# kaushik87599/Melo-GAN

Measured on AMD Instinct MI355X. Metric: piano-roll samples/sec (G+D step), batch=64 128x256 roll, higher is better.
Workload: dtype f32; 1 GPU; cfg2: 128x256 piano-roll, batch=64 per GPU, full G+D+emotion-D step (1 critic update incl. gradient penalty + 1 generator update); global_batch=64, T=256, C=128, parallelism=dp1, graph=True

## Files before the change

### include/melo_gan_hip.h

```cpp
#ifndef MELO_GAN_HIP_H
#define MELO_GAN_HIP_H

#include <stddef.h>
#include <stdint.h>

#ifdef __cplusplus
extern "C" {
#endif

typedef void* mg_stream_t;

enum { MG_ACT_NONE = 0, MG_ACT_RELU = 1, MG_ACT_LRELU = 2, MG_ACT_GELU = 3, MG_ACT_TANH = 4 };

typedef struct mg_epilogue {
    const float* bias;
    const float* scale;
    const float* shift;
    float* zout;
    int act;
    const float* gref;
    int gact;
    const float* emul;
    const float* gscale;
    int accumulate;
// ... 12 lines not shown
                       int B, int Tin, int Cin, int N, int Tout,
                       int w_sn, int w_sc, long xbs, long ybs,
                       const mg_epilogue* epi, void* work, size_t work_bytes, mg_stream_t stream);

int mg_wq_relayout(const float* w, float* wq, int N, int Cc, int K, int w_sn, int w_sc, mg_stream_t stream);
int mg_conv16_supported(int B, int Tin, int Cin, int N, int transposed, int Tout);
int mg_conv16_plan(int B, int Tin, int N, int transposed, int* batch_rows_per_tile, int* part_rows, int* tile_rows);
int mg_conv16_poolable(int B, int Tin, int Cin, int N);
typedef struct mg_conv16_extra {
    float* part;
    float* pool;
    float pool_scale;
    int y_perm;
    const float* mix_real;
    const float* mix_alpha;
    float* mix_out;
    int mix_rows;
    const float* bnb_a;
    const float* bnb_z;
    const float* bnb_mean;
    const float* bnb_invstd;
    double* bnb_part;
    int bnb_act;
} mg_conv16_extra;
int mg_conv16(const float* x, const float* wq, float* y, int B, int Tin, int Cin, int N, int transposed, int Tout,
              long xbs, long ybs, const mg_epilogue* epi, const mg_conv16_extra* extra , mg_stream_t stream);
int mg_bn_train_bwd_parts(const double* part, int part_rows, const float* da, const float* a, const float* z, float* dz, long R,
                          int C, const float* gamma, const float* beta, const float* save_mean, const float* save_invstd,
                          float* dgamma, float* dbeta, int act, mg_stream_t stream);
int mg_bn_train_fwd_parts(const float* part, int part_rows_per_group, int groups, const float* z, float* a, long R, int C,
                          const float* gamma, const float* beta, float* running_mean, float* running_var, float momentum,
                          float eps, float* save_mean, float* save_invstd, int act, mg_stream_t stream);

#define MG_CHAIN_MAX_OPS 16
#define MG_CHAIN_SLOTS 6
#define MG_CHAIN_MAX_VEC 512
enum { MG_CH_LOAD = 1, MG_CH_STORE = 2, MG_CH_LAYERNORM = 3, MG_CH_LIN_FWD = 4, MG_CH_LIN_DGRAD = 5, MG_CH_SOFTMAX_CE = 6,
       MG_CH_DHEAD = 7, MG_CH_MEAN_T = 8, MG_CH_COPY = 9 };
typedef struct mg_chain_op {
    int kind;
    int a, b;
    int n0, n1;
    int act;
    int i0, i1;
    float f0;
    const float* p0; long ld0;
    const float* p1; long ld1;
// ... 347 lines not shown
```

### melo-gan_amd/_lib.py

```python
import ctypes as C
import os

_HERE = os.path.dirname(os.path.abspath(__file__))
LIB_PATH = os.path.join(_HERE, "libmelogan_hip.so")
if os.environ.get("MELO_LIB_VARIANT"):
    LIB_PATH = os.path.join(os.path.dirname(_HERE), "tools", "_build", "libmelogan_" + os.environ["MELO_LIB_VARIANT"] + ".so")

ACT_NONE, ACT_RELU, ACT_LRELU, ACT_GELU, ACT_TANH = 0, 1, 2, 3, 4

vp, i32, i64, f32, sz = C.c_void_p, C.c_int, C.c_long, C.c_float, C.c_size_t


class Epilogue(C.Structure):
    _fields_ = [("bias", vp), ("scale", vp), ("shift", vp), ("zout", vp), ("act", i32),
                ("gref", vp), ("gact", i32), ("emul", vp), ("gscale", vp), ("accumulate", i32)]


class EpilogueBf16(C.Structure):
    _fields_ = [("scale", vp), ("shift", vp), ("zout", vp), ("act", i32), ("gref", vp), ("gact", i32), ("gscale", vp),
                ("accumulate", i32)]


class Conv16Extra(C.Structure):
    _fields_ = [("part", vp), ("pool", vp), ("pool_scale", f32), ("y_perm", i32), ("mix_real", vp), ("mix_alpha", vp),
                ("mix_out", vp), ("mix_rows", i32), ("bnb_a", vp), ("bnb_z", vp), ("bnb_mean", vp), ("bnb_invstd", vp),
                ("bnb_part", vp), ("bnb_act", i32)]


class ChainOp(C.Structure):
    _fields_ = [("kind", i32), ("a", i32), ("b", i32), ("n0", i32), ("n1", i32), ("act", i32), ("i0", i32), ("i1", i32), ("f0", f32),
                ("p0", vp), ("ld0", i64), ("p1", vp), ("ld1", i64), ("p2", vp), ("ld2", i64), ("p3", vp), ("ld3", i64),
                ("q0", vp), ("lq0", i64), ("q1", vp), ("lq1", i64), ("t0", vp)]


CH_LOAD, CH_STORE, CH_LAYERNORM, CH_LIN_FWD, CH_LIN_DGRAD, CH_SOFTMAX_CE, CH_DHEAD, CH_MEAN_T, CH_COPY = 1, 2, 3, 4, 5, 6, 7, 8, 9
CHAIN_MAX_OPS, CHAIN_SLOTS, CHAIN_MAX_VEC = 16, 6, 512


class StageJob(C.Structure):
    _fields_ = [("src", vp), ("dst", vp), ("idx", vp), ("row_bytes", i64), ("src_rows", i64), ("dst_pitch", i64), ("rows", i64)]


MAX_STAGE_JOBS = 8


class Augment(C.Structure):
    _fields_ = [("program", i32), ("noise_std", f32), ("dropout_prob", f32), ("pitch_shift_prob", f32), ("tempo_jitter", f32),
                ("note_dropout", f32), ("velocity_jitter", f32), ("timing_jitter", f32), ("pitch_shift", i32), ("seed", C.c_uint64)]

# ... 37 lines not shown

class Voice(C.Structure):
    _fields_ = [("n_partials", i32), ("mult", C.c_uint32 * VOICE_MAX_PARTIALS), ("weight", f32 * VOICE_MAX_PARTIALS),
                ("decay", f32 * VOICE_MAX_PARTIALS), ("attack", i32), ("release_tau", f32), ("release_len", i32), ("fs", f32)]


class MlpCls(C.Structure):
    _fields_ = [("n_hidden", i32), ("in_dim", i32), ("width", i32 * MLP_MAX_HIDDEN), ("n_classes", i32),
                ("w", vp * (MLP_MAX_HIDDEN + 1)), ("b", vp * (MLP_MAX_HIDDEN + 1)), ("z", vp * MLP_MAX_HIDDEN),
                ("a", vp * MLP_MAX_HIDDEN), ("dz", vp * MLP_MAX_HIDDEN), ("mask", vp * MLP_MAX_HIDDEN)]


SIGNATURES = {
    "mg_version": (i32, []),
    "mg_last_error": (C.c_char_p, []),
    "mg_conv_workspace_bytes": (sz, [i32, i32, i32]),
    "mg_conv1d_gather": (i32, [vp, vp, vp, i32, i32, i32, i32, i32, i32, i32, i32, i32, i64, i64, C.POINTER(Epilogue), vp, sz, i64, vp]),
    "mg_conv1d_scatter2": (i32, [vp, vp, vp, i32, i32, i32, i32, i32, i32, i32, i64, i64, C.POINTER(Epilogue), vp, sz, vp]),
    "mg_wq_relayout": (i32, [vp, vp, i32, i32, i32, i32, i32, vp]),
    "mg_conv16_supported": (i32, [i32, i32, i32, i32, i32, i32]),
    "mg_conv16_plan": (i32, [i32, i32, i32, i32, C.POINTER(i32), C.POINTER(i32), C.POINTER(i32)]),
    "mg_conv16": (i32, [vp, vp, vp, i32, i32, i32, i32, i32, i32, i64, i64, C.POINTER(Epilogue), C.POINTER(Conv16Extra), vp]),
    "mg_conv16_poolable": (i32, [i32, i32, i32, i32]),
    "mg_bn_train_fwd_parts": (i32, [vp, i32, i32, vp, vp, i64, i32, vp, vp, vp, vp, f32, f32, vp, vp, i32, vp]),
    "mg_linear_workspace_bytes": (sz, [i32, i32, i32]),
    "mg_linear": (i32, [vp, vp, vp, i32, i32, i32, i32, i32, C.POINTER(Epilogue), i32, vp, sz, vp]),
    "mg_conv_tile_config": (i32, [i64, i32, i32]),
    "mg_conv_plan": (i32, [i32, i32, i32, i32, i32, i32, i32, i32, sz, C.POINTER(i32), C.POINTER(i32)]),
    "mg_conv_finish_vec": (i32, [i32, i64, i32]),
    "mg_linear_route": (i32, [i32, i32, i32, i32, i32, i32, i32, i32, C.POINTER(i32), C.POINTER(i32), C.POINTER(i32)]),
    "mg_conv_thin_route": (i32, [vp, i64, i32, i32, i32, i32, i32]),
    "mg_wb_relayout": (i32, [vp, vp, i32, i32, i32, i32, i32, i32, vp]),
    "mg_conv1d_s1_bf16_supported": (i32, [i32, i32, i32, i32, i32]),
    "mg_conv1d_s1_bf16": (i32, [vp, i32, vp, vp, i32, i32, i32, i32, i32, i32, C.POINTER(EpilogueBf16), vp]),
    "mg_meanT_fwd_bf16": (i32, [vp, vp, i32, i32, i32, vp]),
    "mg_meanT_bwd_bf16": (i32, [vp, vp, vp, i32, vp, i32, i32, i32, vp]),
    "mg_wgrad_workspace_bytes": (sz, [i32, i32, i32, i32, i32]),
    "mg_wgrad": (i32, [vp, vp, i32, vp, vp, i32, vp, vp, i32, i32, i32, i32, i32, i32, i32, vp, sz, vp]),
    "mg_wgrad_multi": (i32, [vp, i32, i32, i32, vp, sz, vp]),
    "mg_colsum_workspace_bytes": (sz, [i32]),
    "mg_colsum": (i32, [vp, i64, i32, vp, vp, vp, sz, vp]),
    "mg_bn_workspace_bytes": (sz, [i32, i32]),
    "mg_bn_train_fwd": (i32, [vp, vp, i64, i32, i32, vp, vp, vp, vp, f32, f32, vp, vp, i32, vp, sz, vp]),
    "mg_bn_train_bwd": (i32, [vp, vp, vp, vp, i64, i32, vp, vp, vp, vp, vp, vp, i32, vp, sz, vp]),
    "mg_bn_train_bwd_parts": (i32, [vp, i32, vp, vp, vp, vp, i64, i32, vp, vp, vp, vp, vp, vp, i32, vp]),
    "mg_bn_eval_fwd": (i32, [vp, vp, i64, i32, vp, vp, vp, vp, f32, i32, vp]),
# ... 134 lines not shown
```

### melo-gan_amd/csrc/conv16_mfma.hip

```cpp
#include "common.h"
#include <stdlib.h>
#include <type_traits>

namespace {

typedef unsigned u32x4 __attribute__((ext_vector_type(4)));

struct Conv16P {
    const float* x;
    const float* wq;
    float* y;
    int B, Tin, Cin, Tm, Tout, N;
    long xbs, ybs;
    int x_bytes, w_bytes;
    int tt_log2, n_ttiles;
    unsigned nt_magic;
    mg_epilogue e;
    float* part;
    float* pool;
    float pool_scale;
    int y_perm;
    const float* mix_real;
    const float* mix_alpha;
    float* mix_out;
    int mix_rows;
    const float* bnb_a;
    const float* bnb_z;
    const float* bnb_mean;
    const float* bnb_invstd;
    double* bnb_part;
    int bnb_act;
};

constexpr int K5 = 5;
constexpr int BKC = 16;
template <bool TR2> struct PitchOf { static constexpr int value = TR2 ? 24 : 20; };
constexpr int BN = 32;
constexpr int WPLANE = BN * 4;
constexpr int WSLAB = 4 * K5 * WPLANE;
constexpr int MAXX = 3;
constexpr int NWU = 3;

template <bool TR2, int RT, bool RID>
__global__ __launch_bounds__(256, 2) void conv16_kernel(const Conv16P p) {
    constexpr int BM = 32 * RT;
    constexpr int SX = PitchOf<TR2>::value;
    constexpr int SA = TR2 ? 1 : 2;
    constexpr int NR = TR2 ? 3 : 5;
    constexpr int NPH = TR2 ? 2 : 1;
    extern __shared__ __attribute__((aligned(16))) float smem[];

    const int tid = threadIdx.x, lane = tid & 63, wave = tid >> 6;
    const int wm = wave >> 1, wn = wave & 1;
    const int li = lane & 15, kq = lane >> 4;
    const int TT = 1 << p.tt_log2, TB = BM >> p.tt_log2;
    const int R = (TT - 1) * SA + NR;
    const int nrows = TB * R;
    const int xs_floats = nrows * SX;
    const int buf_floats = xs_floats + WSLAB;

    const int mtile = blockIdx.x;
    int mq = (int)__umulhi((unsigned)mtile, p.nt_magic);
    if ((mq + 1) * p.n_ttiles <= mtile) ++mq;
    const int b0 = mq * TB;
    const int t0 = (mtile - mq * p.n_ttiles) * TT;
    const int n0 = blockIdx.y * BN;
    const int tin0 = TR2 ? (t0 - 1) : (2 * t0 - 2);

    auto lds4 = [&](int off) { return reinterpret_cast<f32x4*>(__builtin_assume_aligned(smem + off, 16)); };

    int abase[RT];
#pragma unroll
    for (int rt = 0; rt < RT; ++rt) {
        const int im = (wm * RT + rt) * 16 + li;
        const int seg = im >> p.tt_log2, tl = im & (TT - 1);
        abase[rt] = (seg * R + tl * SA) * SX + 4 * kq;
    }
    const int bbase = xs_floats + kq * K5 * WPLANE + (16 * wn + li) * 4;

    constexpr int KA = RT == 1 ? 2 : 1;
    f32x4 acc[NPH][RT][KA];
#pragma unroll
    for (int ph = 0; ph < NPH; ++ph)
#pragma unroll
        for (int rt = 0; rt < RT; ++rt)
#pragma unroll
            for (int ka = 0; ka < KA; ++ka) acc[ph][rt][ka] = f32x4{0.f, 0.f, 0.f, 0.f};

    const __amdgpu_buffer_rsrc_t xrsrc = __builtin_amdgcn_make_buffer_rsrc(const_cast<float*>(p.x), 0, p.x_bytes, 0x00020000);
    const __amdgpu_buffer_rsrc_t wrsrc = __builtin_amdgcn_make_buffer_rsrc(const_cast<float*>(p.wq), 0, p.w_bytes, 0x00020000);
    const int sink = 2 * buf_floats + 4 * tid;
    constexpr int NST = MAXX + NWU;
    unsigned so[NST];
    int sl[NST], sd[NST];
#pragma unroll
    for (int j = 0; j < MAXX; ++j) {
        const int idx = tid + 256 * j;
        so[j] = 0x80000000u;
        sl[j] = sink;
        sd[j] = 0;
        if (idx < nrows * 4) {
            const int row = idx >> 2, q = idx & 3;
            const int seg = (TB == 1) ? 0 : row / R, r = row - seg * R;
            const int b = b0 + seg, tin = tin0 + r;
            sl[j] = row * SX + 4 * q;
            sd[j] = buf_floats;
            if (b < p.B && tin >= 0 && tin < p.Tin)
                so[j] = ((unsigned)b * (unsigned)p.xbs + (unsigned)(tin * p.Cin + 4 * q)) * 4u;
        }
    }
#pragma unroll
    for (int i = 0; i < NWU; ++i) {
        const int u = tid + 256 * i;
        so[MAXX + i] = 0x80000000u;
        sl[MAXX + i] = sink;
        sd[MAXX + i] = 0;
        if (u < 4 * K5 * BN) {
            const int pl = u >> 5, n = u & 31;
            sl[MAXX + i] = xs_floats + u * 4;
            sd[MAXX + i] = buf_floats;
            if (n0 + n < p.N) so[MAXX + i] = ((unsigned)pl * (unsigned)p.N + (unsigned)(n0 + n)) * 16u;
        }
    }
    const unsigned wchunk = (unsigned)(K5 * p.N) * 16u;
    f32x4 sr[NST];
    auto bload = [&](const __amdgpu_buffer_rsrc_t& rsrc, unsigned voff, unsigned soff) {
        const u32x4 v = __builtin_amdgcn_raw_buffer_load_b128(rsrc, voff, soff, 0);
// ... 51 lines not shown
#pragma unroll
        for (int u = 0; u < NST; ++u) store_unit(u, 0);
        const int c1 = min(BKC, c_last);
#pragma unroll
        for (int u = 0; u < NST; ++u) load_unit(u, 4u * (unsigned)c1, (unsigned)(c1 >> 2) * wchunk);
        __syncthreads();
#pragma unroll
        for (int g = 0; g < NFR; ++g) frag_piece(0, 0, g, fa[0], fb[0]);
    }
    for (int c0 = 0;;) {
        chunk(std::integral_constant<int, 0>{}, min(c0 + 2 * BKC, c_last));
        c0 += BKC;
        if (c0 >= p.Cin) break;
        chunk(std::integral_constant<int, 1>{}, min(c0 + 2 * BKC, c_last));
        c0 += BKC;
        if (c0 >= p.Cin) break;
    }

    const mg_epilogue& E = p.e;
    const int n = n0 + 16 * wn + li;
    if (n >= p.N) return;
    const float bias = E.bias ? E.bias[n] : 0.f;
    const float scale = E.scale ? E.scale[n] : 1.f, shift = E.scale ? E.shift[n] : 0.f;
    const float gscale = E.gscale ? E.gscale[n] : 1.f;
    float st1 = 0.f, cnt = 0.f;
    double bs1 = 0.0, bs2 = 0.0;
    const float bnb_mu = (RID && p.bnb_part) ? p.bnb_mean[n] : 0.f, bnb_is = (RID && p.bnb_part) ? p.bnb_invstd[n] : 0.f;
    const bool want_stats = RID && (p.part || p.pool);
#pragma unroll
    for (int rt = 0; rt < RT; ++rt)
#pragma unroll
        for (int ph = 0; ph < NPH; ++ph) {
            f32x4 a = acc[ph][rt][0];
            if constexpr (KA == 2) a += acc[ph][rt][1];
            unsigned di[4], yi[4];
            bool ok[4], mixrow[4];
            int brow[4];
#pragma unroll
            for (int r = 0; r < 4; ++r) {
                const int im = (wm * RT + rt) * 16 + 4 * kq + r;
                const int seg = im >> p.tt_log2, tl = im & (TT - 1);
                const int b = b0 + seg, t = t0 + tl;
                const int tout = TR2 ? 2 * t + ph : t;
                di[r] = (unsigned)((b * p.Tout + tout) * p.N + n);
                yi[r] = (unsigned)(b * (int)p.ybs + ((RID && p.y_perm) ? n * p.Tout + tout : tout * p.N + n));
                ok[r] = b < p.B && t < p.Tm && tout < p.Tout;
// ... 111 lines not shown
            float m2 = 0.f;
#pragma unroll
            for (int rt = 0; rt < RT; ++rt)
#pragma unroll
                for (int ph = 0; ph < NPH; ++ph)
#pragma unroll
                    for (int r = 0; r < 4; ++r) {
                        const int im = (wm * RT + rt) * 16 + 4 * kq + r;
                        const int seg = im >> p.tt_log2, tl = im & (TT - 1);
                        const int b = b0 + seg, t = t0 + tl;
                        const int tout = TR2 ? 2 * t + ph : t;
                        const float d = acc[ph][rt][0][r] - mw;
                        if (b < p.B && t < p.Tm && tout < p.Tout) m2 += d * d;
                    }
            m2 += __shfl_xor(m2, 16, 64); m2 += __shfl_xor(m2, 32, 64);
            if (kq == 0) {
                float* dst = p.part + (long)(2 * blockIdx.x + wm) * 3 * p.N + n;
                dst[0] = st1;
                dst[p.N] = m2;
                dst[2 * p.N] = cnt;
            }
        }
    }
}

__global__ void wq_relayout_kernel(const float* __restrict__ w, float* __restrict__ wq, int N, int Cc, int K, int sn, int sc) {
    const long i = (long)blockIdx.x * blockDim.x + threadIdx.x;
    if (i >= (long)N * Cc * K) return;
    const int e = (int)(i & 3);
    const long r = i >> 2;
    const int n = (int)(r % N);
    const long r2 = r / N;
    const int k = (int)(r2 % K), q = (int)(r2 / K);
    wq[i] = w[(long)n * sn + (long)(4 * q + e) * sc + k];
}

template <bool TR2, int RT, bool RID>
int launch16(Conv16P p, hipStream_t stream) {
    constexpr int BM = 32 * RT;
    constexpr int SX = PitchOf<TR2>::value;
    constexpr int SA = TR2 ? 1 : 2;
    constexpr int NR = TR2 ? 3 : 5;
    int lg = mg_ilog2_ceil(p.Tm);
    const int lgbm = mg_ilog2_ceil(BM);
    if (lg > lgbm) lg = lgbm;
    p.tt_log2 = lg;
    const int TT = 1 << lg, TB = BM >> lg;
    p.n_ttiles = (int)mg_cdiv(p.Tm, TT);
    p.nt_magic = p.n_ttiles > 1 ? (unsigned)((1ULL << 32) / (unsigned)p.n_ttiles) : 0xFFFFFFFFu;
    const int R = (TT - 1) * SA + NR;
    if (TB * R * 4 > 256 * MAXX) return MG_EUNSUP;
    const size_t lds = 2 * ((size_t)TB * R * SX + WSLAB) * sizeof(float) + 256 * 4 * sizeof(float);
    auto kernel = &conv16_kernel<TR2, RT, RID>;
    static std::atomic<uint64_t> optin;
    if (int rc = mg_lds_optin(reinterpret_cast<const void*>(kernel), optin)) return rc;
    dim3 grid((unsigned)(p.n_ttiles * mg_cdiv(p.B, TB)), (unsigned)mg_cdiv(p.N, BN));
    hipLaunchKernelGGL(kernel, grid, dim3(256), lds, stream, p);
    MG_CHECK_LAUNCH("conv16");
    return MG_OK;
}

}

extern "C" int mg_wq_relayout(const float* w, float* wq, int N, int Cc, int K, int w_sn, int w_sc, mg_stream_t stream) {
    MG_CHECK_ARG(w && wq && N > 0 && Cc > 0 && K > 0 && Cc % 4 == 0 && w_sn > 0 && w_sc > 0, "mg_wq_relayout: bad args");
    const long total = (long)N * Cc * K;
    hipLaunchKernelGGL(wq_relayout_kernel, dim3((unsigned)mg_cdiv(total, 256)), dim3(256), 0, (hipStream_t)stream, w, wq, N, Cc, K,
                       w_sn, w_sc);
    MG_CHECK_LAUNCH("wq_relayout");
    return MG_OK;
}

static int pick_rt(long m_rows, int N) {
    if (const char* f = getenv("MG_CONV16_RT")) return atoi(f) == 1 ? 1 : 2;
    auto balance = [](long n) { return n >= 1024 ? 1.0 : (double)n / (double)(mg_cdiv(n, 256) * 256); };
    const long n2 = mg_cdiv(m_rows, 64) * mg_cdiv(N, BN), n1 = mg_cdiv(m_rows, 32) * mg_cdiv(N, BN);
    return balance(n1) > balance(n2) + 0.1 ? 1 : 2;
}

extern "C" int mg_conv16_supported(int B, int Tin, int Cin, int N, int transposed, int Tout) {
    if (B <= 0 || Tin <= 0 || Cin % BKC || N % BN) return 0;
    const int Tm = transposed ? Tin : (Tin + 4 - K5) / 2 + 1;
    if (Tm < 4) return 0;
    if (transposed && !(Tout == 2 * Tin || Tout == 2 * Tin - 1)) return 0;
// ... 4 lines not shown
    if (lg > mg_ilog2_ceil(BM)) lg = mg_ilog2_ceil(BM);
    const int TT = 1 << lg, TB = BM >> lg, R = (TT - 1) * (transposed ? 1 : 2) + (transposed ? 3 : 5);
    return TB * R * 4 <= 256 * MAXX;
}

extern "C" int mg_conv16_plan(int B, int Tin, int N, int transposed, int* batch_rows_per_tile, int* part_rows, int* tile_rows) {
    const int Tm = transposed ? Tin : (Tin + 4 - K5) / 2 + 1;
    const int BM = 32 * pick_rt((long)B * Tm, N);
    int lg = mg_ilog2_ceil(Tm);
    if (lg > mg_ilog2_ceil(BM)) lg = mg_ilog2_ceil(BM);
    const int TT = 1 << lg, TB = BM >> lg;
    if (batch_rows_per_tile) *batch_rows_per_tile = TB;
    if (tile_rows) *tile_rows = BM;
    if (part_rows) *part_rows = 2 * (int)(mg_cdiv(Tm, TT) * mg_cdiv(B, TB));
    return MG_OK;
}

extern "C" int mg_conv16_poolable(int B, int Tin, int Cin, int N) {
    if (!mg_conv16_supported(B, Tin, Cin, N, 0, 0)) return 0;
    const int Tm = (Tin + 4 - K5) / 2 + 1;
    return Tm == 16 * pick_rt((long)B * Tm, N);
}

extern "C" int mg_conv16(const float* x, const float* wq, float* y, int B, int Tin, int Cin, int N, int transposed, int Tout,
                         long xbs, long ybs, const mg_epilogue* epi, const mg_conv16_extra* extra, mg_stream_t stream) {
    const mg_conv16_extra ex = extra ? *extra : mg_conv16_extra{};
    float* const part = ex.part;
    float* const pool = ex.pool;
    const float pool_scale = ex.pool_scale;
    MG_CHECK_ARG(x && wq && y, "mg_conv16: null tensor");
    MG_CHECK_ARG(!(part && epi && epi->accumulate), "mg_conv16: statistics of an accumulating launch are not defined");
    MG_CHECK_ARG(!(pool && epi && epi->accumulate), "mg_conv16: the mean of an accumulating launch is not defined");
    MG_CHECK_ARG(!pool || (!transposed && mg_conv16_poolable(B, Tin, Cin, N)), "mg_conv16: shape is not poolable");
    MG_CHECK_ARG(!ex.mix_out || (ex.mix_real && ex.mix_alpha && ex.mix_rows > 0 && ex.mix_rows <= B && !ex.y_perm),
                 "mg_conv16: mix needs real, alpha, 0 < rows <= B and the plain output order");
    MG_CHECK_ARG(!ex.y_perm || (ybs == 0 || ybs == (long)N * (transposed ? Tout : (Tin + 4 - K5) / 2 + 1)),
                 "mg_conv16: the permuted output order needs a dense y");
    const int Tm = transposed ? Tin : (Tin + 4 - K5) / 2 + 1;
    if (!transposed) Tout = Tm;
    MG_CHECK_ARG(mg_conv16_supported(B, Tin, Cin, N, transposed, Tout), "mg_conv16: unsupported shape B=%d Tin=%d Cin=%d N=%d", B, Tin, Cin, N);
    Conv16P p{};
    p.x = x; p.wq = wq; p.y = y;
    p.B = B; p.Tin = Tin; p.Cin = Cin; p.Tm = Tm; p.Tout = Tout; p.N = N;
    p.xbs = xbs ? xbs : (long)Tin * Cin;
    p.ybs = ybs ? ybs : (long)Tout * N;
    const long xb = ((long)(B - 1) * p.xbs + (long)Tin * Cin) * 4, yb = (long)(B - 1) * p.ybs + (long)Tout * N;
    MG_CHECK_ARG(xb < (1L << 31) && yb < (1L << 31) && p.ybs < (1L << 31), "mg_conv16: tensor exceeds the 2^31 limit");
    p.x_bytes = (int)xb;
    p.w_bytes = (int)((long)N * Cin * K5 * 4);
// ... 31 lines not shown
```

### melo-gan_amd/gan/engine.py

```python
from __future__ import annotations

import math
import os
from collections import OrderedDict
from typing import Optional, Sequence

import torch

from .. import ops
from ..ops import ACT_GELU, ACT_LRELU, ACT_RELU
from ..emotion_discriminator.layers import tail_bwd, tail_fwd
from ..params import (BN_EPS, BN_MOM, P_DROP, FlatParams, discriminator_spec, emotion_disc_spec, feature_encoder_spec,
                      generator_spec, norm_buffers)
from .ema import ema_config

Tensor = torch.Tensor
ED_SIDE_LDS_PAD = 42000


class GanEngine:

    def __init__(self, cfg: dict, ed_cfg: dict, device="cuda", batch_size: Optional[int] = None, ed_dtype: str = "fp32"):
        if ed_dtype not in ("fp32", "bf16"):
            raise ValueError(f"ed_dtype={ed_dtype!r}: expected 'fp32' or 'bf16'")
# ... 186 lines not shown
        self._chain_gf = (self._chain_e and Ch.supported(self.in_dim, 512, max(self.latent_dim, 1)) and self.latent_dim % 4 == 0
                          and Ch.weights_ok(PG("noise_to_latent.net.0.weight"), PG("noise_to_latent.net.2.weight"),
                                            PG("decoder.pre.0.weight")))
        self._chain_d = on and Ch.supported(256, self.E) and Ch.weights_ok(PD["fc.1.weight"])
        mh = tuple(self.ed_cfg.get("mlp_hidden", (256, 128)))
        ws = [PED[f"classifier.net.{3 * j}.weight"] for j in range(len(mh))] + [PED["classifier.head.weight"]]
        dims = list(mh) + [self.ed_feat_dim]
        n_ops = 2 * (len(mh) + 1) + 3
        if self.ed_mode == "notes":
            ws.append(PED["encoder.project.weight"])
            dims.append(self.ed_pool.shape[1])
            n_ops += 2
        self._chain_ed = (on and self.n_classes <= 32 and Ch.supported(*dims) and Ch.weights_ok(*ws) and
                          n_ops <= ops.L.CHAIN_MAX_OPS)
        self.ed_loss_rows = torch.zeros(self.B, device=self.dev)
        self._gin_done = False

    def params_changed(self):
        for fp, name, t, N, Cc, sn, sc in self._wq_src:
            ops.wq_relayout(fp.p[name], t, N, Cc, 5, sn, sc)
        self.fold_ed()

    class _Riders:
        __slots__ = ("parts", "pooled", "perm", "mixed", "bnb")

        def __init__(self):
            self.parts, self.pooled, self.perm, self.mixed, self.bnb = None, False, False, False, None

    def _conv5s2(self, kind: str, x: Tensor, fp: "FlatParams", name: str, y: Tensor, stats=None, pool=None, perm=False,
                 mix=None, bnb=None, **epi):
        w = fp.p[name]
        res = GanEngine._Riders()
        transposed = kind in ("conv_dgrad", "convT_fwd")
        direction = "fwd" if kind.endswith("fwd") else "dgrad"
        N = w.shape[0] if kind in ("conv_fwd", "convT_dgrad") else w.shape[1]
        wq = self.wq.get((name, direction))
        B, Tin, Cin = x.shape
        Ty = y.shape[2] if perm else y.shape[1]
        odd = transposed and Ty == 2 * Tin - 1 and kind == "conv_dgrad"
        if wq is not None and ops.conv16_supported(B, Tin, Cin, N, transposed, (2 * Tin - (1 if odd else 0)) if transposed else 0):
            kw = dict(epi)
            if pool is not None and kind == "conv_fwd" and ops.conv16_poolable(B, Tin, Cin, N):
                kw["pool"] = (pool, 1.0 / y.shape[1])
                res.pooled = True
            if stats is not None:
                tb, rows = ops.conv16_plan(B, Tin, N, transposed)
                if stats % tb == 0:
                    part = ops.workspace(12 * rows * N, x.device, "bn_part").view(torch.float32)
                    kw["stats"] = part
                    res.parts = (part, rows)
            if perm:
                kw["perm"] = res.perm = True
            if bnb is not None and y.shape[1] == (2 * Tin if transposed else (Tin + 4 - 5) // 2 + 1):
                rows = ops.conv16_plan(B, Tin, N, transposed)[1]
                bpart = ops.workspace(16 * rows * N, x.device, "bnb_part").view(torch.float64)
                kw["bnb"] = (bnb[0], bnb[1], bnb[2], bnb[3], bpart, bnb[4])
                res.bnb = (bpart, rows)
            if mix is not None:
                kw["mix"] = mix
                res.mixed = True
            ops.conv16(x, wq, y, N, transposed, odd=odd, **kw)
            return res
        if perm:
            return res
# ... 270 lines not shown
            mix = (self.real, self.alpha, self.X0[:self.B], self.B)
        self._conv5s2("convT_fwd", v("a_d3"), self.GE, "G.decoder.deconv.6.weight", out, mix=mix, bias=P("decoder.deconv.6.bias"))
        if train:
            self.num_batches_tracked += n // self.B

    def _bn(self, z, a, name, i, train, which="g", parts=None):
        P = self._gp
        if train:
            groups = 2 if which == "both" else 1
            g0 = 0 if which in ("d", "both") else 1
            mean = self.bn_mean_2[i] if groups == 2 else self.bn_mean_2[i][g0]
            invstd = self.bn_invstd_2[i] if groups == 2 else self.bn_invstd_2[i][g0]
            if parts is not None:
                ops.bn_train_fwd_parts(parts[0], parts[1], groups, z, a, P(name + ".weight"), P(name + ".bias"),
                                       self.Gbuf[name + ".running_mean"], self.Gbuf[name + ".running_var"], mean, invstd,
                                       ACT_RELU, self.bn_mom, BN_EPS)
                return
            ops.bn_train_fwd(z, a, P(name + ".weight"), P(name + ".bias"), self.Gbuf[name + ".running_mean"],
                             self.Gbuf[name + ".running_var"], mean, invstd, ACT_RELU, self.bn_mom, BN_EPS, groups=groups)
        else:
            ops.bn_eval_fwd(z, a, P(name + ".weight"), P(name + ".bias"), self.Gbuf[name + ".running_mean"],
                            self.Gbuf[name + ".running_var"], ACT_RELU, BN_EPS)

    def _d_fwd(self, x: Tensor, nb: int, emb: Tensor, head: bool = True):
        P = self.D.p
        self._conv5s2("conv_fwd", x, self.D, "conv.0.weight", self.A1[:nb], bias=P["conv.0.bias"], act=ACT_LRELU)
        self._conv5s2("conv_fwd", self.A1[:nb], self.D, "conv.2.weight", self.A2[:nb], bias=P["conv.2.bias"], act=ACT_LRELU)
        if not self._conv5s2("conv_fwd", self.A2[:nb], self.D, "conv.4.weight", self.A3[:nb], pool=self.H[:nb],
                             bias=P["conv.4.bias"], act=ACT_LRELU).pooled:
            ops.meanT_fwd(self.A3[:nb], self.H[:nb])
        if self._chain_d and not head:
            return
        ops.linear_fwd(self.H[:nb], P["fc.1.weight"], self.Fh[:nb], bias=P["fc.1.bias"], act=ACT_LRELU)
        if head:
            ops.dhead_fwd(self.Fh[:nb], emb, P["real_fake.weight"].view(-1), P["real_fake.bias"], self.s[:nb])

    def _d_bwd_input(self, ds: Tensor, nb: int, emb: Tensor, demb: Optional[Tensor], with_head: bool = False, mean=None):
        P = self.D.p
        if with_head and self._chain_d and (demb is None or emb.shape[0] == nb):
            ch = ops.Chain(nb)
            ch.load(0, self.H[:nb])
            ch.linear_fwd(0, 1, P["fc.1.weight"], P["fc.1.bias"], ACT_LRELU, out=self.Fh[:nb])
            ch.dhead(1, 2, P["real_fake.weight"].view(-1), P["real_fake.bias"], emb, ds, self.s[:nb], demb=demb)
            ch.store(2, self.dU[:nb])
            ch.linear_dgrad(2, 3, P["fc.1.weight"], out=self.dH[:nb])
            ch.launch()
        else:
            if with_head and self._chain_d:
                ops.linear_fwd(self.H[:nb], P["fc.1.weight"], self.Fh[:nb], bias=P["fc.1.bias"], act=ACT_LRELU)
# ... 80 lines not shown

    def _ed_bwd_convs(self, dnotes: Tensor, mean=None, lds_pad: int = 0):
        last = len(self.ed_chans) - 1
        if self.ed_dtype == "bf16":
            ops.meanT_bwd_bf16(self.ed_dpool, self.ed_dz[last], self.ed_z[last], ACT_GELU, self.ed_scale[last])
            for i in range(last, 0, -1):
                ops.conv_s1_bf16(self.ed_dz[i], self.ed_wb_d[i], self.ed_dz[i - 1], gref=self.ed_z[i - 1], gact=ACT_GELU,
                                 gscale=self.ed_scale[i - 1])
            ops.conv_s1_bf16(self.ed_dz[0], self.ed_wb_d[0], dnotes)
            return
        ops.meanT_bwd(self.ed_dpool, self.ed_dz[last], gref=self.ed_z[last], gact=ACT_GELU, gscale=self.ed_scale[last], mean=mean)
        for i in range(last, 0, -1):
            self._ed_conv_dgrad(i, self.ed_dz[i - 1], lds_pad)
        self._ed_conv_dgrad(0, dnotes, lds_pad)

    def d_backward(self, forward: bool = True, side=None):
        B = self.B
        P, G = self.D.p, self.D.g
        if forward:
            self._e_fwd(True, "d", gin=True)
            self._g_fwd(self.fake_d, True, "d")
        if not self._mix_fused:
            ops.gp_interp(self.real, self.fake_d, self.alpha, self.X0[:B])
        self._d_fwd(self.X0[:3 * B], 3 * B, self.emb_d, head=False)
        self._d_bwd_input(self.ds_d, 3 * B, self.emb_d, None, with_head=True)
        self._conv5s2("conv_dgrad", self.dZ1[:B], self.D, "conv.0.weight", self.gx)
        ops.gp_penalty(self.gx, self.TAN0, self.norms, None, self.lambda_gp)
        self._conv5s2("conv_fwd", self.TAN0, self.D, "conv.0.weight", self.TAN1, gref=self.A1[:B], gact=ACT_LRELU)
        self._conv5s2("conv_fwd", self.TAN1, self.D, "conv.2.weight", self.TAN2, gref=self.A2[:B], gact=ACT_LRELU)
        tz3_pooled = self._conv5s2("conv_fwd", self.TAN2, self.D, "conv.4.weight", self.TZ3, pool=self.ghb, gref=self.A3[:B],
                                   gact=ACT_LRELU).pooled
        wjobs = [
            ops.conv1d_wgrad(self.X0[B:3 * B], self.dZ1[B:], G["conv.0.weight"], 2, self.TAN0, self.dZ1[:B],
                             db=G["conv.0.bias"], defer=True),
            ops.conv1d_wgrad(self.A1[B:], self.dZ2[B:], G["conv.2.weight"], 2, self.TAN1, self.dZ2[:B],
                             db=G["conv.2.bias"], defer=True),
            ops.conv1d_wgrad(self.A2[B:], self.dZ3[B:], G["conv.4.weight"], 2, self.TAN2, self.dZ3[:B],
                             db=G["conv.4.bias"], defer=True)]
        if side is not None:
            side.wait_stream(torch.cuda.current_stream())
            with torch.cuda.stream(side):
                ops.wgrad_multi(wjobs)
                self._d_wgrad_ev = torch.cuda.Event()
                self._d_wgrad_ev.record(side)
        else:
            ops.wgrad_multi(wjobs)
        if not tz3_pooled:
# ... 353 lines not shown
```

### melo-gan_amd/ops.py

```python
from __future__ import annotations

import ctypes as C
import functools
import math
from typing import NamedTuple, Optional

import torch

from . import _lib as L
from ._lib import ACT_NONE, ACT_RELU, ACT_LRELU, ACT_GELU, ACT_TANH, Epilogue

Tensor = torch.Tensor


def _stream() -> C.c_void_p:
    return C.c_void_p(torch.cuda.current_stream().cuda_stream)


def _p(t: Optional[Tensor]):
    return None if t is None else C.c_void_p(t.data_ptr())


def _chk(t: Tensor, name: str, shape=None, dtype=torch.float32):
    if not isinstance(t, torch.Tensor) or not t.is_cuda:
# ... 221 lines not shown
    Cin, Cout, K = w.shape
    if dy.shape[2] != Cout:
        raise ValueError("convT1d_dgrad: channel mismatch")
    return conv_gather(dy, w, dx, Cin, K, 2, Cout * K, K, **epi)


def wq_relayout(w: Tensor, wq: Tensor, N: int, Cc: int, K: int, w_sn: int, w_sc: int) -> Tensor:
    _chk(w, "w")
    _chk(wq, "wq")
    if wq.numel() != N * Cc * K or w.numel() < (N - 1) * w_sn + (Cc - 1) * w_sc + K or Cc % 4:
        raise ValueError("wq_relayout: size mismatch")
    L.check(L.load().mg_wq_relayout(_p(w), _p(wq), N, Cc, K, w_sn, w_sc, _stream()), "mg_wq_relayout")
    return wq


def conv16_supported(B: int, Tin: int, Cin: int, N: int, transposed: bool, Tout: int = 0) -> bool:
    return bool(L.load().mg_conv16_supported(B, Tin, Cin, N, 1 if transposed else 0, Tout))


def conv16_poolable(B: int, Tin: int, Cin: int, N: int) -> bool:
    return bool(L.load().mg_conv16_poolable(B, Tin, Cin, N))


def conv16_pool(x: Tensor, wq: Tensor, y: Tensor, N: int, pool: Tensor, scale: float, **epi) -> Tensor:
    return conv16(x, wq, y, N, False, pool=(pool, scale), **epi)


def conv16_plan(B: int, Tin: int, N: int, transposed: bool):
    return _conv16_plan(B, Tin, N, transposed)[:2]


def _conv16_plan(B, Tin, N, transposed):
    tb, rows, bm = C.c_int(), C.c_int(), C.c_int()
    L.check(L.load().mg_conv16_plan(B, Tin, N, 1 if transposed else 0, C.byref(tb), C.byref(rows), C.byref(bm)), "mg_conv16_plan")
    return tb.value, rows.value, bm.value


def conv16(x: Tensor, wq: Tensor, y: Tensor, N: int, transposed: bool, odd: bool = False, stats=None, pool=None,
           perm: bool = False, mix=None, bnb=None, **epi) -> Tensor:
    _chk(x, "x")
    _chk(wq, "wq")
    _chk(y, "y")
    B, Tin, Cin = x.shape
    Tout = (2 * Tin - (1 if odd else 0)) if transposed else (Tin + 4 - 5) // 2 + 1
    if perm:
        if tuple(y.shape) != (B, N, Tout):
            raise ValueError(f"y (perm): expected {(B, N, Tout)}, got {tuple(y.shape)}")
        Ty = Tout
    else:
        if y.dim() != 3 or y.shape[0] != B or y.shape[2] != N or y.shape[1] < Tout:
            raise ValueError(f"y: expected (B={B}, >={Tout}, {N}), got {tuple(y.shape)}")
        Ty = y.shape[1]
    if wq.numel() != N * Cin * 5:
        raise ValueError(f"wq: numel {wq.numel()} != {N * Cin * 5}")
    e = epilogue((B, Tout, N), N, **epi)
    if Ty != Tout and (e.zout or e.gref or e.emul):
        raise ValueError("padded y cannot be combined with elementwise epilogue tensors")
    lib = L.load()
    if not lib.mg_conv16_supported(B, Tin, Cin, N, 1 if transposed else 0, Tout):
        raise ValueError(f"conv16: unsupported shape B={B} Tin={Tin} Cin={Cin} N={N}")
    ex = L.Conv16Extra()
    if stats is not None:
        part = _chk(stats, "stats")
        if part.numel() < 3 * conv16_plan(B, Tin, N, transposed)[1] * N:
            raise ValueError("conv16: partial-statistics buffer too small (conv16_plan)")
# ... 21 lines not shown
        real, alpha, out, rows = mix
        if perm or not 0 < rows <= B:
            raise ValueError("conv16: mix needs the plain output order and 0 < rows <= B")
        for nm, t in (("mix real", real), ("mix out", out)):
            _chk(t, nm)
            if t.dim() != 3 or t.shape[0] < rows or tuple(t.shape[1:]) != (Ty, N):
                raise ValueError(f"conv16: {nm} must be (>= {rows}, {Ty}, {N}), got {tuple(t.shape)}")
        _chk(alpha, "mix alpha")
        if alpha.numel() < rows:
            raise ValueError("conv16: mix alpha has fewer entries than rows")
        ex.mix_real, ex.mix_alpha, ex.mix_out, ex.mix_rows = _p(real), _p(alpha), _p(out), int(rows)

    def launch():
        return lib.mg_conv16(_p(x), _p(wq), _p(y), B, Tin, Cin, N, 1 if transposed else 0, Tout, Tin * Cin, Ty * N, C.byref(e),
                             C.byref(ex), _stream())
    rid = "true" if (stats is not None or pool is not None or perm or mix is not None or bnb is not None) else "false"
    sym = lambda: "conv16_kernel<%s,%d,%s>" % ("true" if transposed else "false", _conv16_plan(B, Tin, N, transposed)[2] // 32, rid)
    with _observe(sym, 2.0 * B * (Tin if transposed else Tout) * N * Cin * 5, launch):
        rc = launch()
    L.check(rc, "mg_conv16")
    return y


SKINNY_MAX_ROWS = 512


def linear_route(M: int, K: int, N: int, w_sn: int, w_sc: int, perm_L: int = 0, x_aligned: bool = True, w_aligned: bool = True):
    lib = L.load()
    kc, vec, ks = C.c_int(), C.c_int(), C.c_int()
    rc = lib.mg_linear_route(M, K, N, w_sn, w_sc, perm_L, int(x_aligned), int(w_aligned), C.byref(kc), C.byref(vec), C.byref(ks))
    if rc < 0:
        L.check(rc, "mg_linear_route")
    if rc == 0:
        return "conv_wgemm_kernel<1,1,false,true,%s>" % {22: "2,2", 12: "1,2", 11: "1,1"}[lib.mg_conv_tile_config(M, N, 0)], 1
    return "linear_skinny_kernel<%s,%s>" % ("true" if kc.value else "false", "true" if vec.value else "false"), ks.value


def _linear(x, w, y, K, N, w_sn, w_sc, epi, perm_L=0):
    M = x.shape[0]
    e = epilogue((M, N), N, **epi)
    lib = L.load()
    need = lib.mg_linear_workspace_bytes(M, N, K)
    work = workspace(need, x.device, "linear") if need else None
    sym = lambda: linear_route(M, K, N, w_sn, w_sc, perm_L, x.data_ptr() % 16 == 0, w.data_ptr() % 16 == 0)[0]
    with _observe(sym, 2.0 * M * N * K):
        rc = lib.mg_linear(_p(x), _p(w), _p(y), M, K, N, w_sn, w_sc, C.byref(e), perm_L, _p(work),
# ... 2236 lines not shown
```

Measured before the change: 79960 samples/s.

## Derive interpolated-sample first D conv from real and fake outputs by linearity

The first discriminator conv used to run over three batches: the real samples, the fakes and the gradient-penalty interpolates. A new lerp variant of the conv16 kernel now convolves only the real/fake pairs. Because the conv plus the bias/affine epilogue is linear, each tile forms the interpolate row's pre-activation as alpha*z_real + (1-alpha)*z_fake, then writes all three activated outputs. This removes a third of the layer's MFMA work and input loads, at the cost of a separate kernel instantiation and a new env-gated code path.

New measurement: 80400 samples/s (median of 6 runs). Within noise of the previous version (+0.5%).

```diff
diff --git a/include/melo_gan_hip.h b/include/melo_gan_hip.h
--- a/include/melo_gan_hip.h
+++ b/include/melo_gan_hip.h
@@ -58,7 +58,10 @@
     const float* bnb_invstd;
     double* bnb_part;
     int bnb_act;
+    const float* lerp_alpha;
+    int lerp_rows, pair_stride;
 } mg_conv16_extra;
+int mg_conv16_lerp_supported(int rows, int Tin, int Cin, int N);
 int mg_conv16(const float* x, const float* wq, float* y, int B, int Tin, int Cin, int N, int transposed, int Tout,
               long xbs, long ybs, const mg_epilogue* epi, const mg_conv16_extra* extra , mg_stream_t stream);
 int mg_bn_train_bwd_parts(const double* part, int part_rows, const float* da, const float* a, const float* z, float* dz, long R,
diff --git a/melo-gan_amd/_lib.py b/melo-gan_amd/_lib.py
--- a/melo-gan_amd/_lib.py
+++ b/melo-gan_amd/_lib.py
@@ -24,7 +24,7 @@
 class Conv16Extra(C.Structure):
     _fields_ = [("part", vp), ("pool", vp), ("pool_scale", f32), ("y_perm", i32), ("mix_real", vp), ("mix_alpha", vp),
                 ("mix_out", vp), ("mix_rows", i32), ("bnb_a", vp), ("bnb_z", vp), ("bnb_mean", vp), ("bnb_invstd", vp),
-                ("bnb_part", vp), ("bnb_act", i32)]
+                ("bnb_part", vp), ("bnb_act", i32), ("lerp_alpha", vp), ("lerp_rows", i32), ("pair_stride", i32)]
 
 
 class ChainOp(C.Structure):
@@ -108,6 +108,7 @@
     "mg_conv16_plan": (i32, [i32, i32, i32, i32, C.POINTER(i32), C.POINTER(i32), C.POINTER(i32)]),
     "mg_conv16": (i32, [vp, vp, vp, i32, i32, i32, i32, i32, i32, i64, i64, C.POINTER(Epilogue), C.POINTER(Conv16Extra), vp]),
     "mg_conv16_poolable": (i32, [i32, i32, i32, i32]),
+    "mg_conv16_lerp_supported": (i32, [i32, i32, i32, i32]),
     "mg_bn_train_fwd_parts": (i32, [vp, i32, i32, vp, vp, i64, i32, vp, vp, vp, vp, f32, f32, vp, vp, i32, vp]),
     "mg_linear_workspace_bytes": (sz, [i32, i32, i32]),
     "mg_linear": (i32, [vp, vp, vp, i32, i32, i32, i32, i32, C.POINTER(Epilogue), i32, vp, sz, vp]),
diff --git a/melo-gan_amd/csrc/conv16_mfma.hip b/melo-gan_amd/csrc/conv16_mfma.hip
--- a/melo-gan_amd/csrc/conv16_mfma.hip
+++ b/melo-gan_amd/csrc/conv16_mfma.hip
@@ -30,6 +30,8 @@
     const float* bnb_invstd;
     double* bnb_part;
     int bnb_act;
+    const float* lerp_alpha;
+    int lerp_rows, pair_stride;
 };
 
 constexpr int K5 = 5;
@@ -41,8 +43,9 @@
 constexpr int MAXX = 3;
 constexpr int NWU = 3;
 
-template <bool TR2, int RT, bool RID>
-__global__ __launch_bounds__(256, 2) void conv16_kernel(const Conv16P p) {
+template <bool TR2, int RT, bool RID, bool LERP>
+__device__ __forceinline__ void conv16_tile(const Conv16P p) {
+    static_assert(!LERP || (!TR2 && RT == 2 && !RID), "the pair tile is the gather form in 64-row tiles, no other rider");
     constexpr int BM = 32 * RT;
     constexpr int SX = PitchOf<TR2>::value;
     constexpr int SA = TR2 ? 1 : 2;
@@ -62,7 +65,7 @@
     const int mtile = blockIdx.x;
     int mq = (int)__umulhi((unsigned)mtile, p.nt_magic);
     if ((mq + 1) * p.n_ttiles <= mtile) ++mq;
-    const int b0 = mq * TB;
+    const int b0 = LERP ? mq : mq * TB;
     const int t0 = (mtile - mq * p.n_ttiles) * TT;
     const int n0 = blockIdx.y * BN;
     const int tin0 = TR2 ? (t0 - 1) : (2 * t0 - 2);
@@ -73,7 +76,7 @@
 #pragma unroll
     for (int rt = 0; rt < RT; ++rt) {
         const int im = (wm * RT + rt) * 16 + li;
-        const int seg = im >> p.tt_log2, tl = im & (TT - 1);
+        const int seg = LERP ? rt : im >> p.tt_log2, tl = LERP ? 16 * wm + li : im & (TT - 1);
         abase[rt] = (seg * R + tl * SA) * SX + 4 * kq;
     }
     const int bbase = xs_floats + kq * K5 * WPLANE + (16 * wn + li) * 4;
@@ -102,7 +105,7 @@
         if (idx < nrows * 4) {
             const int row = idx >> 2, q = idx & 3;
             const int seg = (TB == 1) ? 0 : row / R, r = row - seg * R;
-            const int b = b0 + seg, tin = tin0 + r;
+            const int b = LERP ? b0 + seg * p.pair_stride : b0 + seg, tin = tin0 + r;
             sl[j] = row * SX + 4 * q;
             sd[j] = buf_floats;
             if (b < p.B && tin >= 0 && tin < p.Tin)
@@ -200,6 +203,45 @@
     if (n >= p.N) return;
     const float bias = E.bias ? E.bias[n] : 0.f;
     const float scale = E.scale ? E.scale[n] : 1.f, shift = E.scale ? E.shift[n] : 0.f;
+    if constexpr (LERP) {
+        const float al = p.lerp_alpha[b0], be = 1.f - al;
+        f32x4 z[2];
+#pragma unroll
+        for (int rt = 0; rt < 2; ++rt) {
+            z[rt] = acc[0][rt][0];
+#pragma unroll
+            for (int r = 0; r < 4; ++r) z[rt][r] = (z[rt][r] + bias) * scale + shift;
+        }
+        f32x4 zh;
+#pragma unroll
+        for (int r = 0; r < 4; ++r) zh[r] = fmaf(al, z[0][r], be * z[1][r]);
+        if (E.act == MG_ACT_RELU) {
+#pragma unroll
+            for (int r = 0; r < 4; ++r) { z[0][r] = mg_act(MG_ACT_RELU, z[0][r]); z[1][r] = mg_act(MG_ACT_RELU, z[1][r]); zh[r] = mg_act(MG_ACT_RELU, zh[r]); }
+        } else if (E.act == MG_ACT_LRELU) {
+#pragma unroll
+            for (int r = 0; r < 4; ++r) { z[0][r] = mg_act(MG_ACT_LRELU, z[0][r]); z[1][r] = mg_act(MG_ACT_LRELU, z[1][r]); zh[r] = mg_act(MG_ACT_LRELU, zh[r]); }
+        } else if (E.act == MG_ACT_GELU) {
+#pragma unroll
+            for (int r = 0; r < 4; ++r) { z[0][r] = mg_act(MG_ACT_GELU, z[0][r]); z[1][r] = mg_act(MG_ACT_GELU, z[1][r]); zh[r] = mg_act(MG_ACT_GELU, zh[r]); }
+        } else if (E.act == MG_ACT_TANH) {
+#pragma unroll
+            for (int r = 0; r < 4; ++r) { z[0][r] = mg_act(MG_ACT_TANH, z[0][r]); z[1][r] = mg_act(MG_ACT_TANH, z[1][r]); zh[r] = mg_act(MG_ACT_TANH, zh[r]); }
+        }
+        const unsigned yh = (unsigned)(b0 * (int)p.ybs), yr = (unsigned)((p.lerp_rows + b0) * (int)p.ybs),
+                       yf = (unsigned)((p.lerp_rows + b0 + p.pair_stride) * (int)p.ybs);
+#pragma unroll
+        for (int r = 0; r < 4; ++r) {
+            const int t = t0 + 16 * wm + 4 * kq + r;
+            if (b0 < p.lerp_rows && t < p.Tm) {
+                const unsigned i = (unsigned)(t * p.N + n);
+                p.y[yr + i] = z[0][r];
+                p.y[yf + i] = z[1][r];
+                p.y[yh + i] = zh[r];
+            }
+        }
+        return;
+    }
     const float gscale = E.gscale ? E.gscale[n] : 1.f;
     float st1 = 0.f, cnt = 0.f;
     double bs1 = 0.0, bs2 = 0.0;
@@ -357,6 +399,15 @@
             }
         }
     }
+}
+
+template <bool TR2, int RT, bool RID>
+__global__ __launch_bounds__(256, 2) void conv16_kernel(const Conv16P p) {
+    conv16_tile<TR2, RT, RID, false>(p);
+}
+
+__global__ __launch_bounds__(256, 2) void conv16_lerp_kernel(const Conv16P p) {
+    conv16_tile<false, 2, false, true>(p);
 }
 
 __global__ void wq_relayout_kernel(const float* __restrict__ w, float* __restrict__ wq, int N, int Cc, int K, int sn, int sc) {
@@ -395,6 +446,21 @@
     return MG_OK;
 }
 
+int launch16_lerp(Conv16P p, hipStream_t stream) {
+    constexpr int SX = PitchOf<false>::value, TT = 32, TB = 2, R = (TT - 1) * 2 + 5;
+    static_assert(TB * R * 4 <= 256 * MAXX, "staging plan");
+    p.tt_log2 = 5;
+    p.n_ttiles = p.Tm / TT;
+    p.nt_magic = p.n_ttiles > 1 ? (unsigned)((1ULL << 32) / (unsigned)p.n_ttiles) : 0xFFFFFFFFu;
+    const size_t lds = 2 * ((size_t)TB * R * SX + WSLAB) * sizeof(float) + 256 * 4 * sizeof(float);
+    static std::atomic<uint64_t> optin;
+    if (int rc = mg_lds_optin(reinterpret_cast<const void*>(&conv16_lerp_kernel), optin)) return rc;
+    dim3 grid((unsigned)(p.n_ttiles * p.lerp_rows), (unsigned)mg_cdiv(p.N, BN));
+    hipLaunchKernelGGL(conv16_lerp_kernel, grid, dim3(256), lds, stream, p);
+    MG_CHECK_LAUNCH("conv16_lerp");
+    return MG_OK;
+}
+
 }
 
 extern "C" int mg_wq_relayout(const float* w, float* wq, int N, int Cc, int K, int w_sn, int w_sc, mg_stream_t stream) {
@@ -445,9 +511,44 @@
     return Tm == 16 * pick_rt((long)B * Tm, N);
 }
 
+extern "C" int mg_conv16_lerp_supported(int rows, int Tin, int Cin, int N) {
+    if (rows <= 0 || !mg_conv16_supported(2 * rows, Tin, Cin, N, 0, 0)) return 0;
+    const int Tm = (Tin + 4 - K5) / 2 + 1;
+    return Tm % 32 == 0 && (long)3 * rows * Tm * N < (1L << 31);
+}
+
 extern "C" int mg_conv16(const float* x, const float* wq, float* y, int B, int Tin, int Cin, int N, int transposed, int Tout,
                          long xbs, long ybs, const mg_epilogue* epi, const mg_conv16_extra* extra, mg_stream_t stream) {
     const mg_conv16_extra ex = extra ? *extra : mg_conv16_extra{};
+    if (ex.lerp_alpha) {
+        MG_CHECK_ARG(x && wq && y, "mg_conv16: null tensor");
+        MG_CHECK_ARG(ex.lerp_rows > 0 && ex.pair_stride >= ex.lerp_rows && (long)ex.pair_stride + ex.lerp_rows <= B,
+                     "mg_conv16: lerp needs 0 < rows <= pair_stride and pair_stride + rows <= B");
+        const bool other = ex.part || ex.pool || ex.y_perm || ex.mix_out || ex.bnb_part;
+        const bool epi_ok = !epi || !(epi->accumulate || epi->gref || epi->emul || epi->zout || epi->gscale);
+        if (transposed || other || !epi_ok || B != ex.pair_stride + ex.lerp_rows || !mg_conv16_lerp_supported(ex.lerp_rows, Tin, Cin, N) ||
+            !mg_conv16_supported(B, Tin, Cin, N, 0, 0)) {
+            mg_set_error("mg_conv16: the lerp rider takes the gather form over whole 32-position tiles with a bias / scale / "
+                         "activation epilogue and no other rider (B=%d Tin=%d Cin=%d N=%d rows=%d)", B, Tin, Cin, N, ex.lerp_rows);
+            return MG_EUNSUP;
+        }
+        Conv16P p{};
+        p.x = x; p.wq = wq; p.y = y;
+        p.B = B; p.Tin = Tin; p.Cin = Cin; p.Tm = p.Tout = (Tin + 4 - K5) / 2 + 1; p.N = N;
+        p.xbs = xbs ? xbs : (long)Tin * Cin;
+        p.ybs = ybs ? ybs : (long)p.Tout * N;
+        const int yrows = ex.lerp_rows + B;
+        const long xb = ((long)(B - 1) * p.xbs + (long)Tin * Cin) * 4, yb = (long)(yrows - 1) * p.ybs + (long)p.Tout * N;
+        MG_CHECK_ARG(xb < (1L << 31) && yb < (1L << 31) && p.ybs < (1L << 31), "mg_conv16: tensor exceeds the 2^31 limit");
+        p.x_bytes = (int)xb;
+        p.w_bytes = (int)((long)N * Cin * K5 * 4);
+        if (epi) {
+            p.e = *epi;
+            MG_CHECK_ARG(!(p.e.scale && !p.e.shift), "epilogue: scale without shift");
+        }
+        p.lerp_alpha = ex.lerp_alpha; p.lerp_rows = ex.lerp_rows; p.pair_stride = ex.pair_stride;
+        return launch16_lerp(p, (hipStream_t)stream);
+    }
     float* const part = ex.part;
     float* const pool = ex.pool;
     const float pool_scale = ex.pool_scale;
diff --git a/melo-gan_amd/gan/engine.py b/melo-gan_amd/gan/engine.py
--- a/melo-gan_amd/gan/engine.py
+++ b/melo-gan_amd/gan/engine.py
@@ -232,13 +232,13 @@
         self.fold_ed()
 
     class _Riders:
-        __slots__ = ("parts", "pooled", "perm", "mixed", "bnb")
+        __slots__ = ("parts", "pooled", "perm", "mixed", "bnb", "lerped")
 
         def __init__(self):
-            self.parts, self.pooled, self.perm, self.mixed, self.bnb = None, False, False, False, None
+            self.parts, self.pooled, self.perm, self.mixed, self.bnb, self.lerped = None, False, False, False, None, False
 
     def _conv5s2(self, kind: str, x: Tensor, fp: "FlatParams", name: str, y: Tensor, stats=None, pool=None, perm=False,
-                 mix=None, bnb=None, **epi):
+                 mix=None, bnb=None, lerp=None, **epi):
         w = fp.p[name]
         res = GanEngine._Riders()
         transposed = kind in ("conv_dgrad", "convT_fwd")
@@ -250,6 +250,10 @@
         odd = transposed and Ty == 2 * Tin - 1 and kind == "conv_dgrad"
         if wq is not None and ops.conv16_supported(B, Tin, Cin, N, transposed, (2 * Tin - (1 if odd else 0)) if transposed else 0):
             kw = dict(epi)
+            if lerp is not None and kind == "conv_fwd" and B == 3 * lerp[1] and ops.conv16_lerpable(lerp[1], Tin, Cin, N):
+                ops.conv16(x[lerp[1]:], wq, y, N, False, lerp=lerp, **kw)
+                res.lerped = True
+                return res
             if pool is not None and kind == "conv_fwd" and ops.conv16_poolable(B, Tin, Cin, N):
                 kw["pool"] = (pool, 1.0 / y.shape[1])
                 res.pooled = True
@@ -566,9 +570,9 @@
             ops.bn_eval_fwd(z, a, P(name + ".weight"), P(name + ".bias"), self.Gbuf[name + ".running_mean"],
                             self.Gbuf[name + ".running_var"], ACT_RELU, BN_EPS)
 
-    def _d_fwd(self, x: Tensor, nb: int, emb: Tensor, head: bool = True):
+    def _d_fwd(self, x: Tensor, nb: int, emb: Tensor, head: bool = True, lerp=None):
         P = self.D.p
-        self._conv5s2("conv_fwd", x, self.D, "conv.0.weight", self.A1[:nb], bias=P["conv.0.bias"], act=ACT_LRELU)
+        self._conv5s2("conv_fwd", x, self.D, "conv.0.weight", self.A1[:nb], lerp=lerp, bias=P["conv.0.bias"], act=ACT_LRELU)
         self._conv5s2("conv_fwd", self.A1[:nb], self.D, "conv.2.weight", self.A2[:nb], bias=P["conv.2.bias"], act=ACT_LRELU)
         if not self._conv5s2("conv_fwd", self.A2[:nb], self.D, "conv.4.weight", self.A3[:nb], pool=self.H[:nb],
                              bias=P["conv.4.bias"], act=ACT_LRELU).pooled:
@@ -695,7 +699,8 @@
             self._g_fwd(self.fake_d, True, "d")
         if not self._mix_fused:
             ops.gp_interp(self.real, self.fake_d, self.alpha, self.X0[:B])
-        self._d_fwd(self.X0[:3 * B], 3 * B, self.emb_d, head=False)
+        lerp = (self.alpha, B) if os.environ.get("MELO_D_LERP", "1") == "1" else None
+        self._d_fwd(self.X0[:3 * B], 3 * B, self.emb_d, head=False, lerp=lerp)
         self._d_bwd_input(self.ds_d, 3 * B, self.emb_d, None, with_head=True)
         self._conv5s2("conv_dgrad", self.dZ1[:B], self.D, "conv.0.weight", self.gx)
         ops.gp_penalty(self.gx, self.TAN0, self.norms, None, self.lambda_gp)
diff --git a/melo-gan_amd/ops.py b/melo-gan_amd/ops.py
--- a/melo-gan_amd/ops.py
+++ b/melo-gan_amd/ops.py
@@ -267,6 +267,10 @@
     return bool(L.load().mg_conv16_poolable(B, Tin, Cin, N))
 
 
+def conv16_lerpable(rows: int, Tin: int, Cin: int, N: int) -> bool:
+    return bool(L.load().mg_conv16_lerp_supported(rows, Tin, Cin, N))
+
+
 def conv16_pool(x: Tensor, wq: Tensor, y: Tensor, N: int, pool: Tensor, scale: float, **epi) -> Tensor:
     return conv16(x, wq, y, N, False, pool=(pool, scale), **epi)
 
@@ -282,10 +286,13 @@
 
 
 def conv16(x: Tensor, wq: Tensor, y: Tensor, N: int, transposed: bool, odd: bool = False, stats=None, pool=None,
-           perm: bool = False, mix=None, bnb=None, **epi) -> Tensor:
+           perm: bool = False, mix=None, bnb=None, lerp=None, **epi) -> Tensor:
     _chk(x, "x")
     _chk(wq, "wq")
     _chk(y, "y")
+    if lerp is not None:
+        return _conv16_lerp(x, wq, y, N, transposed, lerp, stats is not None or pool is not None or perm or mix is not None
+                            or bnb is not None, epi)
     B, Tin, Cin = x.shape
     Tout = (2 * Tin - (1 if odd else 0)) if transposed else (Tin + 4 - 5) // 2 + 1
     if perm:
@@ -353,6 +360,39 @@
     return y
 
 
+def _conv16_lerp(x, wq, y, N, transposed, lerp, other_rider, epi):
+    alpha, rows = lerp
+    rows = int(rows)
+    B, Tin, Cin = x.shape
+    Tout = (Tin + 4 - 5) // 2 + 1
+    if rows <= 0 or B != 2 * rows:
+        raise ValueError(f"conv16: lerp needs x = [real | fake] of 2 * rows batch rows, got B={B} rows={rows}")
+    if y.dim() != 3 or y.shape[0] < 3 * rows or y.shape[2] != N or y.shape[1] < Tout:
+        raise ValueError(f"y (lerp): expected (>={3 * rows}, >={Tout}, {N}), got {tuple(y.shape)}")
+    if wq.numel() != N * Cin * 5:
+        raise ValueError(f"wq: numel {wq.numel()} != {N * Cin * 5}")
+    _chk(alpha, "lerp alpha")
+    if alpha.numel() < rows:
+        raise ValueError("conv16: lerp alpha has fewer entries than rows")
+    e = epilogue((B, Tout, N), N, **epi)
+    lib = L.load()
+    ex = L.Conv16Extra()
+    ex.lerp_alpha, ex.lerp_rows, ex.pair_stride = _p(alpha), rows, rows
+    if other_rider:
+        ex.y_perm = 1
+
+    def launch():
+        return lib.mg_conv16(_p(x), _p(wq), _p(y), B, Tin, Cin, N, 1 if transposed else 0, 0, Tin * Cin, y.shape[1] * N, C.byref(e),
+                             C.byref(ex), _stream())
+    if (transposed or other_rider or e.zout or e.gref or e.emul or e.gscale or e.accumulate
+            or not lib.mg_conv16_lerp_supported(rows, Tin, Cin, N)):
+        L.check(launch() or -1, "mg_conv16")
+    with _observe(lambda: "conv16_lerp_kernel", 2.0 * B * Tout * N * Cin * 5, launch):
+        rc = launch()
+    L.check(rc, "mg_conv16")
+    return y
+
+
 SKINNY_MAX_ROWS = 512
 
 
```
